# huakunyang/SummerTTS

Measured on AMD Instinct MI355X. Metric: audio samples/sec (acoustic model + vocoder, phoneme ids -> int16 PCM on host), single_speaker_fast-shaped synthetic blob, higher is better.
Workload: dtype f32 (decoder trunk convs AND the reverse flow's WaveNet convs (wn_flow.hip, one-utterance calls): fp32 operands as 2 fp16 terms = 22-23 of their 24 mantissa bits, 3 fp16 MFMA products per fp32 product, f32 accumulation -- measured error in `parity`, same tolerance as the exact-fp32 leg; batches addi

## Files before the change

summertts_amd/csrc/capi.hip:

```cpp
#include <stdlib.h>
#include <string.h>

#include <algorithm>
#include <new>
#include <string>
#include <vector>

#include "engine.hpp"
#include "eq_stream.hpp"
#include "join_stream.hpp"
#include "loud_stream.hpp"

using namespace sts;

struct sts_engine { Engine eng; };

static thread_local std::string g_err;
static int set_err(int code, const std::string& s) { g_err = s; return code; }

extern "C" {

const char* sts_last_error(void) { return g_err.c_str(); }
void sts_free(void* p) { free(p); }

// ... 643 lines not shown
    return STS_OK;
}
int sts_set_record_taps(sts_engine* e, int enable) { if (!e) return set_err(STS_EINVAL, "null engine"); e->eng.record_taps = enable != 0; return STS_OK; }
int sts_set_conv_math(sts_engine* e, int mode) {
    if (!e) return set_err(STS_EINVAL, "null engine");
    if (mode < 0 || mode > 3) return set_err(STS_EINVAL, "conv math: 0 = split-bf16 (default), 1 = exact fp32, 2 = split-bf16 wherever eligible, 3 = two-term fp16");
    e->eng.conv_math = mode;
    e->eng.h2_consecutive = 0; e->eng.h2_disabled = false;
    return STS_OK;
}
int sts_set_conv_mode(sts_engine* e, int mode) { if (!e) return set_err(STS_EINVAL, "null engine"); e->eng.conv_mode = mode; return STS_OK; }
int sts_debug_set(sts_engine* e, int key, int value) {
    if (!e) return set_err(STS_EINVAL, "null engine");
    switch (key) {
        case STS_DBG_ATTN_BLOCK_MIN_WGS: if (value < 1) return set_err(STS_EINVAL, "threshold must be >= 1"); e->eng.attn_block_min_wgs = value; return STS_OK;
        case STS_DBG_FLOW_FUSED: e->eng.flow_fused = value != 0; return STS_OK;
        case STS_DBG_LAUNCH_AHEAD: if (value < 0 || value > 2) return set_err(STS_EINVAL, "launch_ahead must be 0, 1 or 2"); if ((value == 2) != (e->eng.launch_ahead == 2)) { e->eng.seen_tf_.clear(); e->eng.seen_order_.clear(); } e->eng.launch_ahead = value; return STS_OK;
        case STS_DBG_H2P: e->eng.h2p = value < 0 ? 0 : (value > 4 ? 4 : value); return STS_OK;
        case STS_DBG_H2P_TILE: e->eng.h2p_tile = value; return STS_OK;
        case STS_DBG_CHAIN_STREAMS: e->eng.chain_streams_dbg = value; return STS_OK;
        case STS_DBG_TAIL_FUSED: e->eng.tail_fused = value != 0; return STS_OK;
        case STS_DBG_UPS_ROWPH: e->eng.ups_rowph = value != 0; return STS_OK;
        case STS_DBG_MEMO_CLEAR: e->eng.seen_tf_.clear(); e->eng.seen_order_.clear(); return STS_OK;
        case STS_DBG_ATTN_REG: e->eng.attn_reg = value != 0; return STS_OK;
        case STS_DBG_DDS_TAIL: e->eng.dds_tail = value != 0; return STS_OK;
        case STS_DBG_PCM_DIRECT: e->eng.pcm_direct = value != 0; return STS_OK;
        case STS_DBG_STREAM_RETRY_STEP: e->eng.stream_retry_step = value < 0 ? -1 : value; return STS_OK;
        case STS_DBG_STREAM_DIRECT: e->eng.stream_direct = value != 0; return STS_OK;
        case STS_DBG_POISON: e->eng.poison = (unsigned)value; return STS_OK;
        default: return set_err(STS_EINVAL, "unknown debug key");
    }
// ... 846 lines not shown
```

summertts_amd/csrc/engine.hip:

```cpp
#include "run_ctx.hpp"
#include <time.h>
#include "knobs.hpp"
#include "../../include/tts_logger.h"

#include <algorithm>
#include <chrono>
#include <math.h>
#include <stdlib.h>
#include <string.h>
#include <thread>

namespace sts {

Engine::~Engine() {
    if (stream) (void)hipStreamSynchronize(stream);
    free_model(model);
    if (arenaT_.base) (void)hipFree(arenaT_.base);
    if (arenaF_.base) (void)hipFree(arenaF_.base);
    if (pinned_) (void)hipHostFree(pinned_);
    if (pinned_pcm_) (void)hipHostFree(pinned_pcm_);
    if (d_rs_table) (void)hipFree(d_rs_table);
    if (loud_host_) (void)hipHostFree(loud_host_);
    if (lim_host_) (void)hipHostFree(lim_host_);
    if (d_eq_) (void)hipFree(d_eq_);
// ... 17 lines not shown
#elif defined(__aarch64__) || defined(__arm__)
    asm volatile("yield" ::: "memory");
#else
    std::this_thread::yield();
#endif
}

int Engine::init(const float* blob, int64_t bytes, int dev) {
    conv_math = default_conv_math();
    int count = 0;
    if (hipGetDeviceCount(&count) != hipSuccess || count <= 0)
        return fail(STS_EDEVICE, "no HIP device visible: the SummerTTS HIP engine needs an AMD GPU (gfx950) -- there is no CPU fallback");
    if (dev < 0 || dev >= count) return fail(STS_EINVAL, "device index out of range");
    device = dev;
    HIPCK(hipSetDevice(dev));
    HIPCK(hipStreamCreateWithFlags(&stream, hipStreamNonBlocking));
    for (auto& e : ev_) HIPCK(hipEventCreate(&e));
    HIPCK(hipEventCreateWithFlags(&ev_fork_, hipEventDisableTiming));
    HIPCK(hipEventCreateWithFlags(&ev_setup_, hipEventDisableTiming));
    for (auto& e : ev_join_) HIPCK(hipEventCreateWithFlags(&e, hipEventDisableTiming));
    {
        int lo = 0, hi = 0;
        (void)hipDeviceGetStreamPriorityRange(&lo, &hi);
        for (int k = 0; k < kAux; k++) {
            int pr = lo + (hi - lo) * k / (kAux > 1 ? kAux - 1 : 1);
            HIPCK(hipStreamCreateWithPriority(&aux_[k], hipStreamNonBlocking, pr));
        }
    }
    cur_ = stream;
    have_events_ = true;
// ... 879 lines not shown
    for (int u : M.up_rate) upS *= u;
    c.upS = upS;
    std::vector<size_t> stage_elems(M.n_up);
    size_t regA = 0, regB = 0;
    { int S = 1; for (int i = 0; i < M.n_up; i++) { S *= M.up_rate[i]; stage_elems[i] = (size_t)(3 + 4 * M.n_resk) * M.ups[i].Cout * Wcap * S;
          if (i & 1) { if (stage_elems[i] > regB) regB = stage_elems[i]; } else { if (stage_elems[i] > regA) regA = stage_elems[i]; } } }
    const long Lsb = c.Lsb = Wcap * upS + B;
    const int sbC = c.sbC = M.conv_post.Cout;
    bool use_ff = flow_fused && conv_mode == 0 && conv_math == 3 && !M.cp.empty() && wnH > 0;
    for (size_t i = 0; i < M.cp.size() && use_ff; i++)
        use_ff = M.cp[i].ff.ok && M.cp[i].wn.H == wnH && M.cp[i].wn.n == c.wnL && M.cp[i].ff.G == M.cp[0].ff.G && M.cp[i].wn.in[0].k == M.cp[0].wn.in[0].k;
    if (use_ff) {
        long tiles = 0;
        if (B == 1) tiles = (Ftot + 31) / 32;
        else for (int b = 0; b < B; b++) tiles += (p_lenF[b] + 31) / 32;
        use_ff = tiles * M.cp[0].ff.G <= 256;
    }
    c.use_ff = use_ff; c.ffG = use_ff ? M.cp[0].ff.G : 0;
    BufF& bf = c.bf;
    const OutChain& oc = c.oc;
    c.Ocap = oc.run[OS_RESAMPLE] ? out_count((long long)Wcap * hop) + B : (long long)Wcap * hop;
    if (c.join) c.Ocap = oc.run[OS_RESAMPLE] ? out_count(c.FJ * hop) + 1 : c.FJ * hop;
    const long long jwin = ss && c.join ? c.js.window_frames() * hop : c.FJ * hop;
    if (ss && c.join) c.Ocap = oc.run[OS_RESAMPLE] ? out_count(jwin) + 4 : jwin;
    if (ss && oc.run[OS_LIMIT] && oc.run[OS_RESAMPLE]) c.Ocap += B;
    pcm_in_host_ = pcm_direct && host_pcm && !ss && B == 1 && !record_taps && pinned_pcm_dev_ && (size_t)c.Ocap * 2 + 256 <= pinned_pcm_cap_ &&
                   (size_t)c.Ocap * 2 <= ((size_t)4 << 20);
    auto layoutF = [&](Arena& A) {
        A.used = 0;
        for (int q = 0; q < 2; q++) {
            bf.ff_h[q] = A.get<float>(use_ff ? (size_t)wnH * Ftot : 1);
// ... 128 lines not shown
                    }
                    A.w_pre = cp.pre.wh2; A.b_pre = cp.pre.bias; A.s_pre = cp.pre.h2_scale;
                    A.w_gate = ff.gate0; A.s_gate = ff.gate0_scale;
                } else {
                    A.h_in = bf.ff_h[(l - 1) & 1]; A.part_in = bf.ff_part[(l - 1) & 1]; A.part_n = G;
                    A.w_gate = w.in[l].wh2; A.s_gate = w.in[l].h2_scale;
                }
                A.part_stride = (long)((size_t)w.H * Ftot);
                A.h_out = bf.ff_h[l & 1]; A.part_out = bf.ff_part[l & 1];
                A.macc = bf.ff_macc[cs]; A.macc_stride = (long)hF; A.macc_init = l == 0;
                A.b_gate = w.in[l].bias;
                if (w.has_cond) { A.ubias = bt.cond_wn + (size_t)l * 2 * w.H * B; A.ubias_ld = B; }
                A.w_c = ff.wc[l]; A.s_c = ff.sc[l]; A.rows_c = ff.rows_c[l]; A.rows_res = ff.rows_res[l];
                A.b_res = ff.b_res[l]; A.b_m = ff.b_m;
                A.ovf = ovf_;
                flow_layer(A, stream);
                if (l == 0 && pend_set >= 0) { cur[x0h] = A.x0_out; pend_set = -1; }
            }
            ConvOpt os; os.epi = EPI_SUB;
            (void)conv_args(cp.post, nullptr, lv1, nullptr, lv1, os, nullptr);
            pend_set = cs; pend_half = x1h;
        }
        if (pend_set >= 0) finish_half(pend_half, pend_set);
        for (int hh = 0; hh < 2; hh++) if (cur[hh] != home[hh]) finish_half(hh, -1);
    } else
    {
    expand_frames(bt.m, Ttot, bt.cum, lvT.seg, lv1.seg, C, bf.z, Ftot, B, maxF, stream, &pnz);
    tap("z_p", bf.z, C, Ftot, Fcount);

    for (int i = M.n_flows - 1; i >= 0; i--) {
        const DCoupling& cp = M.cp[i];
// ... 502 lines not shown
```

summertts_amd/csrc/engine.hpp:

```cpp
#pragma once
#include <hip/hip_runtime.h>

#include <deque>
#include <map>
#include <unordered_map>
#include <string>
#include <vector>

#include "../../include/summertts_hip.h"
#include "kernels.hpp"
#include "model.hpp"

namespace sts {

struct Arena {
    char* base = nullptr; size_t cap = 0, used = 0; bool measuring = false;
    void* alloc(size_t bytes) {
        size_t a = (used + 255) & ~(size_t)255;
        used = a + bytes;
        if (measuring) return nullptr;
        return base + a;
    }
    template <typename T> T* get(size_t count) { return (T*)alloc(count * sizeof(T)); }
};
// ... 98 lines not shown
    long ahead_misses = 0;
    static constexpr size_t kMemoEntries = 1024;
    std::unordered_map<unsigned long long, long> seen_tf_; std::deque<unsigned long long> seen_order_;
    bool polite_wait = false;
    struct WaitEst { double us = 0.0; long phonemes = 0; };
    WaitEst wait_est_[2][24];
    void nap_before_wait(int which, long phonemes);
    void note_wait(int which, long phonemes, double waited_us, bool was_ready_at_wake);
    int final_sync(long phonemes);
    int ups_rowph = 1;
    int tail_fused = 1;
    int chain_streams_dbg = -1;
    int h2p = 1;
    int h2p_tile = -1;
    int flow_fused = 1;
    int stream_retry_step = -1;
    int stream_direct = 0;
    unsigned poison = 0;
    int64_t poison_bytes_ = 0;
    hipStream_t stream = nullptr;

private:
    int fail(int code, const std::string& msg) { err_ = msg; return code; }
    bool ensure(Arena& a, size_t bytes);
    bool ensure_pinned(size_t bytes);
    void poison_arena(const Arena& a);
    void poison_host16(void* p, size_t samples);
    void poison_host32(void* p, size_t words);
    ConvArgs conv_args(const DConv& c, const float* x, const Lvl& lin, float* y, const Lvl& lout, const ConvOpt& o, double* flops);
    void conv(const DConv& c, const float* x, const Lvl& lin, float* y, const Lvl& lout, const ConvOpt& o);
// ... 60 lines not shown
```

summertts_amd/csrc/kernels.hpp:

```cpp
#pragma once
#include <hip/hip_runtime.h>
#include <stdint.h>

#include <vector>

#include "../../include/summertts_hip.h"

namespace sts {

struct SegView {
    const int* off;
    const int* len;
    int scale;
    int extra;
    int ioff, ilen;
};

enum Epilogue : int {
    EPI_STORE = 0,
    EPI_RESADD = 1,
    EPI_SUB = 3,
    EPI_GATE = 4,
    EPI_RESSKIP = 5,
    EPI_TANH_PCM = 6,
// ... 103 lines not shown
    float* part_out;
    float* macc; long macc_stride; int macc_init;
    const void* w_gate; const float* b_gate; float s_gate;
    const float* ubias; int ubias_ld;
    const void* w_c; float s_c; int rows_c, rows_res;
    const float* b_res; const float* b_m;
    unsigned* ovf;
};
struct FlowFinishArgs {
    SegView seg; int B, max_len; int half;
    const float* src; long src_ld; float* dst; long dst_ld;
    const float* macc; int n; long macc_stride;
};
bool flow_layer_shape_ok(int H, int half, int k, int dil, int n_layers);
int flow_layer_groups(int H);
void flow_layer(const FlowLayerArgs& a, hipStream_t st);
void flow_finish(const FlowFinishArgs& a, hipStream_t st);

bool conv_mfma_eligible(const ConvArgs& a);
void conv_mfma(const ConvArgs& a, hipStream_t st, int tile = -1);
constexpr int kMaxGroup = 4;
struct ConvGroup { ConvArgs g[kMaxGroup]; int n; };
struct ResLayerArgs {
    const float* x; float* y;
    const float *w1, *b1, *w2, *b2;
    int k1, dil1, k2;
    const float *wu1, *wu2;
    const void *wb1, *wb2;
    float ws1, ws2;
};
struct ResLayerGroup {
// ... 239 lines not shown
```

summertts_amd/csrc/run_ctx.hpp:

```cpp
#pragma once
#include "engine.hpp"
#include "eq_stream.hpp"
#include "loud_stream.hpp"
#include "out_chain.hpp"
#include "join_stream.hpp"

namespace sts {

#define HIPCK(call)                                                                           \
    do {                                                                                      \
        hipError_t e__ = (call);                                                              \
        if (e__ != hipSuccess) return fail(STS_EDEVICE, std::string(#call) + ": " + hipGetErrorString(e__)); \
    } while (0)

struct BufT {
    int *meta_i; float* ls; float *ns, *nsw; uint64_t* seed; int* ids; int* forced;
    float *x, *qkv, *att, *y, *x1, *ffh, *m, *logs;
    float *dh, *dt1, *dt2, *dc, *dhh, *dp29, *dr[4], *dlogw;
    int *dur, *cum, *frames;
    float *g, *cond_dp, *cond_dec, *cond_wn;
    float* plan_rate; int *plan_fixed, *plan_target; long long* plan_rem; float* dur_w;
    int* mix;
    int *gain_q, *gain_h;
    int* join_sil;
// ... 42 lines not shown
    int *pm = nullptr, *p_offT = nullptr, *p_lenT = nullptr, *p_sid = nullptr, *p_offF = nullptr, *p_lenF = nullptr, *p_one = nullptr;
    int *d_offT = nullptr, *d_lenT = nullptr, *d_sid = nullptr, *d_offF = nullptr, *d_lenF = nullptr, *d_one = nullptr, *d_win = nullptr;
    bool inl = false, no_inline_seg = false, ms = false;
    long Ftot = 0; int maxF = 0, hop = 0;
    long Fld = 0; int maxFld = 0; bool ahead = false, ahead_b = false, mapped = false, forced = false;
    bool plan = false;
    bool gain = false;
    bool join = false;
    long long FJ = 0;
    bool mix = false;
    std::vector<Engine::Noise> nz; bool any_ns = false, any_nsw = false;
    std::vector<unsigned long long> req_keys; std::vector<long> predF;
    int halo = 0; long Wcap = 0; int upS = 1; long Lsb = 0; int sbC = 0;
    long long Ocap = 0;
    bool bstream = false;
    bool use_ff = false; int ffG = 0;
    OutChain oc{}; LimiterDesign limd; int rsP = 1, rsQ = 1, eqS = 0;
    const float* stage_out(int s) const {
        const float* const o[OS_COUNT] = {bf.wave, bf.wave_gain, bf.wave_join, bf.wave_out, nullptr, bf.wave_eq, nullptr, bf.wave_lim};
        return s < 0 ? nullptr : o[s];
    }
    JsPlan js;
};
#define RUN_ALIASES(c)                                                                                                              \
    [[maybe_unused]] Model& M = model;                                                                                              \
    [[maybe_unused]] const int B = (c).B; [[maybe_unused]] const StreamSpec* const ss = (c).ss;                                     \
    [[maybe_unused]] const long Ttot = (c).Ttot; [[maybe_unused]] const int maxT = (c).maxT;                                        \
    [[maybe_unused]] const int H = (c).H, C = (c).C, FF = (c).FF, fdp = (c).fdp, wnH = (c).wnH, wnL = (c).wnL, ffn2_slices = (c).ffn2_slices; \
    [[maybe_unused]] Lvl &lvT = (c).lvT, &lvB = (c).lvB, &lv1 = (c).lv1;                                                            \
    [[maybe_unused]] BufT& bt = (c).bt; [[maybe_unused]] BufF& bf = (c).bf;                                                         \
    [[maybe_unused]] const size_t up_bytes = (c).up_bytes;                                                                          \
// ... 12 lines not shown
```

summertts_amd/csrc/wn_flow.hip:

```cpp
#include "conv_bf3_dev.hpp"

namespace sts {

#ifdef STS_TILE_TRACE
int tile_trace_bind_flow(long long* buf, unsigned capacity_records) { return tile_trace_bind(buf, capacity_records); }
#endif

constexpr int FL_WIN = 64;
constexpr int FL_NT = 32;
constexpr int FL_UR = 2;
constexpr int FL_MAXG = 8;

__device__ __forceinline__ unsigned fl_b_off(int chunk, int pos, int half, int plane, int plane_bytes) {
    return (unsigned)(chunk * 2 * plane_bytes + plane * plane_bytes + pos * 32 + ((half ^ ((pos >> 3) & 1)) << 4));
}

__device__ __forceinline__ void split4h(const float (&x)[4], unsigned (&hi)[2], unsigned (&lo)[2], float& amax) {
#pragma unroll
    for (int d = 0; d < 2; d++) {
        const f32x2 v = {x[2 * d], x[2 * d + 1]};
        const f16x2 h = __builtin_convertvector(v, f16x2);
#if STS_SPLIT_MIX
        const f32x2 v2 = v * 2048.f;
        const unsigned hu = __builtin_bit_cast(unsigned, h);
// ... 3 lines not shown
            : "+v"(l) : "v"(hu), "s"(-2048.0f), "v"(v2[0]), "v"(v2[1]));
        hi[d] = hu;
        lo[d] = l;
#else
        const f32x2 r = (v - __builtin_convertvector(h, f32x2)) * 2048.f;
        const f16x2 l = __builtin_convertvector(r, f16x2);
        hi[d] = __builtin_bit_cast(unsigned, h);
        lo[d] = __builtin_bit_cast(unsigned, l);
#endif
        amax = __builtin_fmaxf(amax, __builtin_fmaxf(__builtin_fabsf(v[0]), __builtin_fabsf(v[1])));
    }
}

constexpr int FL_WAVES = 8;
constexpr int FL_GSTEPS = 16;
template <bool L0>
__global__ __launch_bounds__(64 * FL_WAVES) __attribute__((amdgpu_waves_per_eu(2, 2))) void flow_layer_kernel(FlowLayerArgs a) {
    extern __shared__ __attribute__((aligned(16))) unsigned char fsm[];
    const int Gp = (a.G + 7) & ~7;
    const int g = (int)(blockIdx.x % (unsigned)Gp);
    if (g >= a.G) return;
    const int rest = (int)(blockIdx.x / (unsigned)Gp);
    const int ntile = (a.max_len + FL_NT - 1) / FL_NT;
    const int b = rest / ntile, tile = rest - b * ntile;
    const int len = uni(seg_len(a.seg, b));
    const int n0 = tile * FL_NT;
    if (n0 >= len) return;
    const size_t base = (size_t)uni(seg_start(a.seg, b));
    const int tid = threadIdx.x, lane = tid & 63, wave = __builtin_amdgcn_readfirstlane(tid >> 6);
    const int l31 = lane & 31, half = lane >> 5;
    const int H = a.H, hc = a.half, Cg = a.Cg, halo = a.halo;
    const int W = FL_NT + 2 * halo;
    const int NCH = H >> 4;
    const int PLANE = FL_WIN * 32;
    unsigned char* const R_h = fsm;
    unsigned char* const R_x = fsm + (size_t)NCH * 2 * PLANE;
    unsigned char* const R_a = R_x + (size_t)FL_WAVES * 4096;
    const int APL = FL_NT * 32;
    float amax = 0.f;
    constexpr int RG = 2, KS = FL_WAVES / RG;
    const int rt_l = wave % RG, kq = wave / RG;
#ifdef STS_TILE_TRACE
    long long* tt_rec = tt_open(3 + (L0 ? 1 : 0), g);
    TT_STAMP(0);
#endif

    const int nrtg = (2 * H) >> 5;
    const int c_lo = NCH * kq / KS, c_hi = NCH * (kq + 1) / KS;
    const int nsteps = (c_hi - c_lo) * a.k;
    u32x4 fa[FL_GSTEPS][1][2];
    auto gate_prefetch = [&](auto lo_c, auto hi_c) {
        constexpr int lo = decltype(lo_c)::value, hi = decltype(hi_c)::value;
        const rsrc_t wrs = make_rsrc(a.w_gate, (unsigned)((size_t)NCH * a.k * nrtg * 2048u));
// ... 22 lines not shown
                    const unsigned off = t < ntc && cs < nkc ? (unsigned)(((g * nkc + cs) * ntc + t) * 2048 + pl * 1024 + lane * 16) : kOOB;
                    fc[ti][cs][0][pl] = __builtin_bit_cast(u32x4, __builtin_amdgcn_raw_buffer_load_b128(wrs, (int)off, 0, 0));
                }
        }
    };

    f32x4u mold[2][4];
    auto m_prefetch = [&]() {
        const rsrc_t rm = make_rsrc(a.macc + (size_t)g * a.macc_stride, a.macc_init ? 0u : (unsigned)(((size_t)a.tot * hc) * 4u));
#pragma unroll
        for (int ti = 0; ti < 2; ti++) {
            const int t = wave + FL_WAVES * ti;
#pragma unroll
            for (int q = 0; q < 4; q++) {
                const int c = t * 32 + 8 * q + 4 * half - a.rows_res;
                const bool okm = t < ntc && c >= 0 && c + 3 < hc && n0 + l31 < len;
                const unsigned off = okm ? (unsigned)(((base + (size_t)(n0 + l31)) * hc + c) * 4u) : kOOB;
                mold[ti][q] = __builtin_bit_cast(f32x4u, __builtin_amdgcn_raw_buffer_load_b128(rm, (int)off, 0, 0));
            }
        }
    };

    if constexpr (!L0) {
        gate_prefetch(I0{}, IH{});
        const int qpp = H >> 2;
        const int nunit = W * qpp;
        const unsigned span = (unsigned)(((size_t)a.tot * H) * 4u);
        const rsrc_t rh = make_rsrc(a.h_in, span);
        for (int u0 = 0; u0 < nunit; u0 += 64 * FL_WAVES * FL_UR) {
            f32x4u v[FL_UR], p[FL_UR][FL_MAXG];
            int pw[FL_UR], q4[FL_UR]; bool ok[FL_UR];
#pragma unroll
            for (int r = 0; r < FL_UR; r++) {
                const int u = u0 + r * 64 * FL_WAVES + tid;
                pw[r] = u / qpp; q4[r] = u - pw[r] * qpp;
                const int pos = n0 - halo + pw[r];
                ok[r] = u < nunit && pos >= 0 && pos < len;
                const unsigned off = ok[r] ? (unsigned)(((base + (size_t)pos) * H + (size_t)q4[r] * 4) * 4u) : kOOB;
                v[r] = __builtin_bit_cast(f32x4u, __builtin_amdgcn_raw_buffer_load_b128(rh, (int)off, 0, 0));
#pragma unroll
                for (int s = 0; s < FL_MAXG; s++) {
                    const rsrc_t rp = make_rsrc(a.part_in + (size_t)s * a.part_stride, s < a.part_n ? span : 0u);
                    p[r][s] = __builtin_bit_cast(f32x4u, __builtin_amdgcn_raw_buffer_load_b128(rp, (int)off, 0, 0));
                }
            }
#pragma unroll
            for (int r = 0; r < FL_UR; r++) {
                const int u = u0 + r * 64 * FL_WAVES + tid;
                if (u >= nunit) continue;
                f32x4u s4 = v[r];
#pragma unroll
                for (int s = 0; s < FL_MAXG; s++) s4 += p[r][s];
                const int ch = q4[r] * 4;
                if (ok[r] && pw[r] >= halo && pw[r] < halo + FL_NT && ch >= g * Cg && ch < (g + 1) * Cg)
                    *(f32x4u*)(a.h_out + (base + (size_t)(n0 - halo + pw[r])) * H + ch) = s4;
                const float x4[4] = {s4[0], s4[1], s4[2], s4[3]};
                unsigned hi[2], lo[2];
                split4h(x4, hi, lo, amax);
                const int chunk = ch >> 4, hf = (ch >> 3) & 1, qd = (ch >> 2) & 1;
                unsigned char* d = R_h + fl_b_off(chunk, pw[r], hf, 0, PLANE) + qd * 8;
                *(uint2*)d = uint2{hi[0], hi[1]};
                *(uint2*)(d + PLANE) = uint2{lo[0], lo[1]};
            }
        }
        TT_STAMP(1);
        gate_prefetch(IH{}, IE{});
        c_prefetch();
        m_prefetch();
    } else {
        gate_prefetch(I0{}, IH{});
        const int nrt = H >> 5, nk = hc >> 4;
        u32x4 fp[8][1][2];
        {
            const rsrc_t wrs = make_rsrc(a.w_pre, (unsigned)((size_t)nk * nrt * 2048u));
#pragma unroll
            for (int cs = 0; cs < 8; cs++)
#pragma unroll
                for (int pl = 0; pl < 2; pl++) {
                    const unsigned o = wave < nrt && cs < nk ? (unsigned)((cs * nrt + wave) * 2048 + pl * 1024 + lane * 16) : kOOB;
                    fp[cs][0][pl] = __builtin_bit_cast(u32x4, __builtin_amdgcn_raw_buffer_load_b128(wrs, (int)o, 0, 0));
                }
        }
        const int qpp = hc >> 2;
        const int nunit = W * qpp;
        const unsigned pspan = (unsigned)(((size_t)a.tot * hc) * 4u);
        for (int u0 = 0; u0 < nunit; u0 += 64 * FL_WAVES * FL_UR) {
            float zv[FL_UR][4]; f32x4u p[FL_UR][FL_MAXG];
            int pw[FL_UR], q4[FL_UR]; bool ok[FL_UR];
#pragma unroll
            for (int r = 0; r < FL_UR; r++) {
                const int u = u0 + r * 64 * FL_WAVES + tid;
                q4[r] = u / W; pw[r] = u - q4[r] * W;
                const int pos = n0 - halo + pw[r];
                ok[r] = u < nunit && pos >= 0 && pos < len;
                const size_t zo = (size_t)(q4[r] * 4) * a.x0_ld + base + (size_t)(ok[r] ? pos : 0);
#pragma unroll
                for (int e = 0; e < 4; e++) zv[r][e] = ok[r] ? a.x0[zo + (size_t)e * a.x0_ld] : 0.f;
                const unsigned off = ok[r] ? (unsigned)(((base + (size_t)pos) * hc + (size_t)q4[r] * 4) * 4u) : kOOB;
#pragma unroll
                for (int s = 0; s < FL_MAXG; s++) {
                    const rsrc_t rp = make_rsrc(a.pend + (size_t)s * a.pend_stride, s < a.pend_n ? pspan : 0u);
                    p[r][s] = __builtin_bit_cast(f32x4u, __builtin_amdgcn_raw_buffer_load_b128(rp, (int)off, 0, 0));
                }
            }
#pragma unroll
            for (int r = 0; r < FL_UR; r++) {
                const int u = u0 + r * 64 * FL_WAVES + tid;
                if (u >= nunit) continue;
                f32x4u s4 = {zv[r][0], zv[r][1], zv[r][2], zv[r][3]};
#pragma unroll
                for (int s = 0; s < FL_MAXG; s++) s4 += p[r][s];
                const int ch = q4[r] * 4;
                if (a.x0_out && ok[r] && pw[r] >= halo && pw[r] < halo + FL_NT && (q4[r] % a.G) == g) {
                    float* zp = a.x0_out + (size_t)ch * a.x0_out_ld + base + (size_t)(n0 - halo + pw[r]);
#pragma unroll
                    for (int e = 0; e < 4; e++) zp[(size_t)e * a.x0_out_ld] = s4[e];
                }
                const float x4[4] = {s4[0], s4[1], s4[2], s4[3]};
                unsigned hi[2], lo[2];
                split4h(x4, hi, lo, amax);
                const int chunk = ch >> 4, hf = (ch >> 3) & 1, qd = (ch >> 2) & 1;
                unsigned char* d = R_x + fl_b_off(chunk, pw[r], hf, 0, PLANE) + qd * 8;
                *(uint2*)d = uint2{hi[0], hi[1]};
                *(uint2*)(d + PLANE) = uint2{lo[0], lo[1]};
            }
        }
        __syncthreads();
        TT_STAMP(1);
        gate_prefetch(IH{}, IE{});
        if (wave < nrt) {
            const int rt = wave;
            f32x16 acc[1][2];
#pragma unroll
            for (int ct = 0; ct < 2; ct++)
#pragma unroll
                for (int r = 0; r < 16; r++) acc[0][ct][r] = 0.f;
#pragma unroll
            for (int cs = 0; cs < 8; cs++)
                if (cs < nk) {
                    u32x4 fb[2][2];
#pragma unroll
                    for (int ct = 0; ct < 2; ct++)
#pragma unroll
                        for (int pl = 0; pl < 2; pl++) fb[ct][pl] = *(const u32x4*)(R_x + fl_b_off(cs, ct * 32 + l31, half, pl, PLANE));
                    step_mfmas<1, 1, 2, 2, 2>(acc, fp[cs], fb);
                }
#pragma unroll
            for (int ct = 0; ct < 2; ct++) {
                const int pw_ = ct * 32 + l31;
                const int pos = n0 - halo + pw_;
                const bool inside = pos >= 0 && pos < len && pw_ < W;
#pragma unroll
                for (int hh = 0; hh < 2; hh++) {
                    float v8[8];
#pragma unroll
                    for (int e = 0; e < 8; e++) {
                        const int row = rt * 32 + hh * 16 + 8 * (e >> 2) + 4 * half + (e & 3);
                        const float t1 = acc[0][ct][hh * 8 + e] * a.s_pre + (a.b_pre ? a.b_pre[row] : 0.f);
                        v8[e] = inside ? t1 : 0.f;
                    }
                    u32x4 ph, pl;
                    split8h(v8, ph, pl, amax);
                    unsigned char* d = R_h + fl_b_off(rt * 2 + hh, pw_, half, 0, PLANE);
                    *(u32x4*)d = ph;
                    *(u32x4*)(d + PLANE) = pl;
                    if (inside && pw_ >= halo && pw_ < halo + FL_NT) {
#pragma unroll
                        for (int qd = 0; qd < 2; qd++) {
                            const int ch = rt * 32 + hh * 16 + 8 * qd + 4 * half;
                            if (ch >= g * Cg && ch < (g + 1) * Cg)
                                *(f32x4u*)(a.h_out + (base + (size_t)pos) * H + ch) = f32x4u{v8[4 * qd], v8[4 * qd + 1], v8[4 * qd + 2], v8[4 * qd + 3]};
                        }
                    }
                }
            }
        }
        c_prefetch();
        m_prefetch();
    }
    __syncthreads();
    TT_STAMP(2);

    f32x16 acc[1][1], acc1[1][1];
#pragma unroll
    for (int r = 0; r < 16; r++) { acc[0][0][r] = 0.f; acc1[0][0][r] = 0.f; }
    {
        u32x4 fb[2][1][2];
        auto load_b = [&](int s, u32x4 (&dst)[1][2]) {
            const int ss = s < nsteps ? s : 0;
            const int c = c_lo + ss / a.k, j = ss - (ss / a.k) * a.k;
// ... 8 lines not shown
                if constexpr (s % 2 == 0) step_mfmas<1, 1, 1, 2, 2>(acc, fa[s], fb[s % 2]);
                else step_mfmas<1, 1, 1, 2, 2>(acc1, fa[s], fb[s % 2]);
            }
        });
#pragma unroll
        for (int r = 0; r < 16; r++) acc[0][0][r] += acc1[0][0][r];
    }
    TT_STAMP(3);
    float* const red = (float*)R_x;
    __syncthreads();
#pragma unroll
    for (int r = 0; r < 16; r++) red[((size_t)(kq * RG + rt_l) * 16 + r) * 64 + lane] = acc[0][0][r];
    __syncthreads();
    {
        const int rowb = (g * RG + rt_l) * 32;
        float gv[2];
#pragma unroll
        for (int i = 0; i < 2; i++) {
            const int r = 2 * kq + i;
            float t = 0.f, sg = 0.f;
            for (int q = 0; q < KS; q++) {
                t += red[((size_t)(q * RG + rt_l) * 16 + r) * 64 + lane];
                sg += red[((size_t)(q * RG + rt_l) * 16 + r + 8) * 64 + lane];
            }
            const int rowp = rowb + (r & 3) + 8 * (r >> 2) + 4 * half;
            t = t * a.s_gate + (a.b_gate ? a.b_gate[rowp] : 0.f);
            sg = sg * a.s_gate + (a.b_gate ? a.b_gate[rowp + 16] : 0.f);
            if (a.ubias) { t += a.ubias[(size_t)rowp * a.ubias_ld + b]; sg += a.ubias[(size_t)(rowp + 16) * a.ubias_ld + b]; }
            gv[i] = tanh_ref(t) * sigmoid_ref(sg);
        }
        const f32x2 v = {gv[0], gv[1]};
        const f16x2 hh = __builtin_convertvector(v, f16x2);
        const f32x2 rr = (v - __builtin_convertvector(hh, f32x2)) * 2048.f;
        const f16x2 ll = __builtin_convertvector(rr, f16x2);
        amax = __builtin_fmaxf(amax, __builtin_fmaxf(__builtin_fabsf(v[0]), __builtin_fabsf(v[1])));
        unsigned char* d = R_a + (size_t)rt_l * 2 * APL + l31 * 32 + ((half ^ ((l31 >> 3) & 1)) << 4) + kq * 4;
        *(unsigned*)d = __builtin_bit_cast(unsigned, hh);
        *(unsigned*)(d + APL) = __builtin_bit_cast(unsigned, ll);
    }
    __syncthreads();
    TT_STAMP(4);

    const int pos_o = n0 + l31;
    const bool col_ok = pos_o < len;
#pragma unroll
    for (int ti = 0; ti < 2; ti++) {
        const int t = wave + FL_WAVES * ti;
        if (t >= ntc) continue;
        f32x16 ac[1][1];
#pragma unroll
        for (int r = 0; r < 16; r++) ac[0][0][r] = 0.f;
#pragma unroll
        for (int cs = 0; cs < 2; cs++)
            if (cs < nkc) {
                u32x4 fb[1][2];
                const unsigned char* sp = R_a + (size_t)cs * 2 * APL + l31 * 32 + ((half ^ ((l31 >> 3) & 1)) << 4);
                fb[0][0] = *(const u32x4*)sp;
                fb[0][1] = *(const u32x4*)(sp + APL);
                step_mfmas<1, 1, 1, 2, 2>(ac, fc[ti][cs], fb);
// ... 32 lines not shown
    const size_t base = (size_t)seg_start(a.seg, b);
    const int idx = blockIdx.x * 256 + threadIdx.x;
    const int qpp = a.half >> 2;
    const int q = idx / a.max_len, pos = idx - q * a.max_len;
    if (q >= qpp || pos >= len) return;
    f32x4u s4;
#pragma unroll
    for (int e = 0; e < 4; e++) s4[e] = a.src[(size_t)(q * 4 + e) * a.src_ld + base + pos];
    for (int s = 0; s < a.n; s++) s4 += *(const f32x4u*)(a.macc + (size_t)s * a.macc_stride + (base + (size_t)pos) * a.half + q * 4);
#pragma unroll
    for (int e = 0; e < 4; e++) a.dst[(size_t)(q * 4 + e) * a.dst_ld + base + pos] = s4[e];
}

bool flow_layer_shape_ok(int H, int half, int k, int dil, int n_layers) {
    if (H < 32 || H % 32 != 0 || H > 256 || half < 16 || half % 16 != 0 || half % 4 != 0 || half > 128) return false;
    if (!(k & 1) || k < 1 || dil != 1 || (k - 1) > FL_WIN - FL_NT || n_layers < 1) return false;
    const int Cg = 32, G = H / Cg;
    if (G > FL_MAXG) return false;
    const int RG = 2, KS = FL_WAVES / RG, NCH = H / 16;
    if (((NCH + KS - 1) / KS) * k > FL_GSTEPS) return false;
    if (half / 16 > 8 || H / 32 > FL_WAVES) return false;
    const int rows_c = ((H + half) + 31) / 32 * 32;
    return rows_c / 32 <= 2 * FL_WAVES;
}
int flow_layer_groups(int H) { return H / 32; }

static size_t flow_lds_bytes(int H) {
    const size_t h = (size_t)(H / 16) * 2 * FL_WIN * 32;
    return h + (size_t)FL_WAVES * 4096 + (size_t)4 * 2 * FL_NT * 32 + 256;
}

void flow_layer(const FlowLayerArgs& a, hipStream_t st) {
    if (a.max_len <= 0 || a.B <= 0) return;
    const int Gp = (a.G + 7) & ~7;
    const int ntile = (a.max_len + FL_NT - 1) / FL_NT;
    const size_t lds = flow_lds_bytes(a.H);
    if (a.layer == 0) {
        (void)hipFuncSetAttribute((const void*)flow_layer_kernel<true>, hipFuncAttributeMaxDynamicSharedMemorySize, (int)lds);
        hipLaunchKernelGGL(flow_layer_kernel<true>, dim3((unsigned)((size_t)ntile * a.B * Gp)), dim3(64 * FL_WAVES), lds, st, a);
    } else {
        (void)hipFuncSetAttribute((const void*)flow_layer_kernel<false>, hipFuncAttributeMaxDynamicSharedMemorySize, (int)lds);
        hipLaunchKernelGGL(flow_layer_kernel<false>, dim3((unsigned)((size_t)ntile * a.B * Gp)), dim3(64 * FL_WAVES), lds, st, a);
    }
}

void flow_finish(const FlowFinishArgs& a, hipStream_t st) {
    if (a.max_len <= 0 || a.B <= 0) return;
    const long n = (long)(a.half >> 2) * a.max_len;
    hipLaunchKernelGGL(flow_finish_kernel, dim3((unsigned)((n + 255) / 256), a.B), dim3(256), 0, st, a);
}

}
```

Baseline: 66.60 million.

## Add 16-column flow layer tiles for small utterances with compact block mapping

Templates the fused WaveNet flow layer kernel on its tile width and adds a 16-column variant. The engine picks it when the live tile count times the group count is at most half the CU count, so short one-utterance calls spread over more workgroups. The 16-wide path uses a denser block-to-(group, tile) mapping that does not waste padded group slots. The partial-sum accumulation loops are also specialised on the actual number of partials, so loads of absent slices are skipped. The cost is a second kernel instantiation and narrower MFMA work per block, which leaves half of each 32-column tile idle and recomputes halo more often.

```diff
diff --git a/summertts_amd/csrc/capi.hip b/summertts_amd/csrc/capi.hip
--- a/summertts_amd/csrc/capi.hip
+++ b/summertts_amd/csrc/capi.hip
@@ -681,7 +681,7 @@
     if (!e) return set_err(STS_EINVAL, "null engine");
     switch (key) {
         case STS_DBG_ATTN_BLOCK_MIN_WGS: if (value < 1) return set_err(STS_EINVAL, "threshold must be >= 1"); e->eng.attn_block_min_wgs = value; return STS_OK;
-        case STS_DBG_FLOW_FUSED: e->eng.flow_fused = value != 0; return STS_OK;
+        case STS_DBG_FLOW_FUSED: e->eng.flow_fused = value == 2 || value == 3 ? value : value != 0; return STS_OK;
         case STS_DBG_LAUNCH_AHEAD: if (value < 0 || value > 2) return set_err(STS_EINVAL, "launch_ahead must be 0, 1 or 2"); if ((value == 2) != (e->eng.launch_ahead == 2)) { e->eng.seen_tf_.clear(); e->eng.seen_order_.clear(); } e->eng.launch_ahead = value; return STS_OK;
         case STS_DBG_H2P: e->eng.h2p = value < 0 ? 0 : (value > 4 ? 4 : value); return STS_OK;
         case STS_DBG_H2P_TILE: e->eng.h2p_tile = value; return STS_OK;
diff --git a/summertts_amd/csrc/engine.hip b/summertts_amd/csrc/engine.hip
--- a/summertts_amd/csrc/engine.hip
+++ b/summertts_amd/csrc/engine.hip
@@ -55,6 +55,7 @@
     if (dev < 0 || dev >= count) return fail(STS_EINVAL, "device index out of range");
     device = dev;
     HIPCK(hipSetDevice(dev));
+    HIPCK(hipDeviceGetAttribute(&n_cus, hipDeviceAttributeMultiprocessorCount, dev));
     HIPCK(hipStreamCreateWithFlags(&stream, hipStreamNonBlocking));
     for (auto& e : ev_) HIPCK(hipEventCreate(&e));
     HIPCK(hipEventCreateWithFlags(&ev_fork_, hipEventDisableTiming));
@@ -964,7 +965,9 @@
         long tiles = 0;
         if (B == 1) tiles = (Ftot + 31) / 32;
         else for (int b = 0; b < B; b++) tiles += (p_lenF[b] + 31) / 32;
-        use_ff = tiles * M.cp[0].ff.G <= 256;
+        if (flow_fused < 2) use_ff = tiles * M.cp[0].ff.G <= 256;
+        const long live = B == 1 ? ((c.ahead && !c.predF.empty() ? c.predF[0] : c.Ftot) + 31) / 32 : tiles;
+        c.ffNT = flow_fused == 3 || (flow_fused == 1 && live * M.cp[0].ff.G <= n_cus / 2) ? 16 : 32;
     }
     c.use_ff = use_ff; c.ffG = use_ff ? M.cp[0].ff.G : 0;
     BufF& bf = c.bf;
@@ -1123,7 +1126,7 @@
                 A.w_c = ff.wc[l]; A.s_c = ff.sc[l]; A.rows_c = ff.rows_c[l]; A.rows_res = ff.rows_res[l];
                 A.b_res = ff.b_res[l]; A.b_m = ff.b_m;
                 A.ovf = ovf_;
-                flow_layer(A, stream);
+                flow_layer(A, stream, c.ffNT);
                 if (l == 0 && pend_set >= 0) { cur[x0h] = A.x0_out; pend_set = -1; }
             }
             ConvOpt os; os.epi = EPI_SUB;
diff --git a/summertts_amd/csrc/engine.hpp b/summertts_amd/csrc/engine.hpp
--- a/summertts_amd/csrc/engine.hpp
+++ b/summertts_amd/csrc/engine.hpp
@@ -136,6 +136,7 @@
     int h2p = 1;
     int h2p_tile = -1;
     int flow_fused = 1;
+    int n_cus = 0;
     int stream_retry_step = -1;
     int stream_direct = 0;
     unsigned poison = 0;
diff --git a/summertts_amd/csrc/kernels.hpp b/summertts_amd/csrc/kernels.hpp
--- a/summertts_amd/csrc/kernels.hpp
+++ b/summertts_amd/csrc/kernels.hpp
@@ -141,7 +141,7 @@
 };
 bool flow_layer_shape_ok(int H, int half, int k, int dil, int n_layers);
 int flow_layer_groups(int H);
-void flow_layer(const FlowLayerArgs& a, hipStream_t st);
+void flow_layer(const FlowLayerArgs& a, hipStream_t st, int nt = 32);
 void flow_finish(const FlowFinishArgs& a, hipStream_t st);
 
 bool conv_mfma_eligible(const ConvArgs& a);
diff --git a/summertts_amd/csrc/run_ctx.hpp b/summertts_amd/csrc/run_ctx.hpp
--- a/summertts_amd/csrc/run_ctx.hpp
+++ b/summertts_amd/csrc/run_ctx.hpp
@@ -80,7 +80,7 @@
     int halo = 0; long Wcap = 0; int upS = 1; long Lsb = 0; int sbC = 0;
     long long Ocap = 0;
     bool bstream = false;
-    bool use_ff = false; int ffG = 0;
+    bool use_ff = false; int ffG = 0, ffNT = 32;
     OutChain oc{}; LimiterDesign limd; int rsP = 1, rsQ = 1, eqS = 0;
     const float* stage_out(int s) const {
         const float* const o[OS_COUNT] = {bf.wave, bf.wave_gain, bf.wave_join, bf.wave_out, nullptr, bf.wave_eq, nullptr, bf.wave_lim};
diff --git a/summertts_amd/csrc/wn_flow.hip b/summertts_amd/csrc/wn_flow.hip
--- a/summertts_amd/csrc/wn_flow.hip
+++ b/summertts_amd/csrc/wn_flow.hip
@@ -6,8 +6,8 @@
 int tile_trace_bind_flow(long long* buf, unsigned capacity_records) { return tile_trace_bind(buf, capacity_records); }
 #endif
 
-constexpr int FL_WIN = 64;
-constexpr int FL_NT = 32;
+constexpr int FL_COLS = 32;
+constexpr int fl_win(int NT) { return NT + 32; }
 constexpr int FL_UR = 2;
 constexpr int FL_MAXG = 8;
 
@@ -41,14 +41,53 @@
 
 constexpr int FL_WAVES = 8;
 constexpr int FL_GSTEPS = 16;
-template <bool L0>
+
+#ifndef STS_FLOW_MAP
+#define STS_FLOW_MAP 0
+#endif
+__host__ __device__ __forceinline__ int flow_grid16(int G, int T) { return STS_FLOW_MAP == 1 ? T * G : 8 * G * ((T + 7) >> 3); }
+template <class F>
+__device__ __forceinline__ void fl_slices(int n, F&& f) {
+    switch (n) {
+        case 0: f(std::integral_constant<int, 0>{}); break;
+        case 1: f(std::integral_constant<int, 1>{}); break;
+        case 2: f(std::integral_constant<int, 2>{}); break;
+        case 3: f(std::integral_constant<int, 3>{}); break;
+        case 4: f(std::integral_constant<int, 4>{}); break;
+        case 5: f(std::integral_constant<int, 5>{}); break;
+        case 6: f(std::integral_constant<int, 6>{}); break;
+        case 7: f(std::integral_constant<int, 7>{}); break;
+        default: f(std::integral_constant<int, 8>{}); break;
+    }
+}
+__device__ __forceinline__ bool flow_block_map(int bid, int G, int T, int& g, int& rest) {
+#if STS_FLOW_MAP == 1
+    rest = bid / G; g = bid - rest * G;
+#else
+    const int c = bid & 7, s = bid >> 3;
+    const int q = s / G, i = s - q * G;
+    if (c < G) { g = c; rest = 8 * q + i; }
+    else {
+        const int m = (c - G) * G + i, sp = 8 - G;
+        g = m / sp; rest = 8 * q + G + (m - g * sp);
+    }
+#endif
+    return rest < T;
+}
+template <bool L0, int NT>
 __global__ __launch_bounds__(64 * FL_WAVES) __attribute__((amdgpu_waves_per_eu(2, 2))) void flow_layer_kernel(FlowLayerArgs a) {
     extern __shared__ __attribute__((aligned(16))) unsigned char fsm[];
-    const int Gp = (a.G + 7) & ~7;
-    const int g = (int)(blockIdx.x % (unsigned)Gp);
-    if (g >= a.G) return;
-    const int rest = (int)(blockIdx.x / (unsigned)Gp);
+    constexpr int FL_NT = NT, FL_WIN = fl_win(NT);
     const int ntile = (a.max_len + FL_NT - 1) / FL_NT;
+    int g, rest;
+    if constexpr (NT == 32) {
+        const int Gp = (a.G + 7) & ~7;
+        g = (int)(blockIdx.x % (unsigned)Gp);
+        if (g >= a.G) return;
+        rest = (int)(blockIdx.x / (unsigned)Gp);
+    } else {
+        if (!flow_block_map((int)blockIdx.x, a.G, ntile * a.B, g, rest)) return;
+    }
     const int b = rest / ntile, tile = rest - b * ntile;
     const int len = uni(seg_len(a.seg, b));
     const int n0 = tile * FL_NT;
@@ -63,7 +102,7 @@
     unsigned char* const R_h = fsm;
     unsigned char* const R_x = fsm + (size_t)NCH * 2 * PLANE;
     unsigned char* const R_a = R_x + (size_t)FL_WAVES * 4096;
-    const int APL = FL_NT * 32;
+    constexpr int APL = FL_COLS * 32;
     float amax = 0.f;
     constexpr int RG = 2, KS = FL_WAVES / RG;
     const int rt_l = wave % RG, kq = wave / RG;
@@ -116,7 +155,7 @@
 #pragma unroll
             for (int q = 0; q < 4; q++) {
                 const int c = t * 32 + 8 * q + 4 * half - a.rows_res;
-                const bool okm = t < ntc && c >= 0 && c + 3 < hc && n0 + l31 < len;
+                const bool okm = t < ntc && c >= 0 && c + 3 < hc && l31 < FL_NT && n0 + l31 < len;
                 const unsigned off = okm ? (unsigned)(((base + (size_t)(n0 + l31)) * hc + c) * 4u) : kOOB;
                 mold[ti][q] = __builtin_bit_cast(f32x4u, __builtin_amdgcn_raw_buffer_load_b128(rm, (int)off, 0, 0));
             }
@@ -129,8 +168,10 @@
         const int nunit = W * qpp;
         const unsigned span = (unsigned)(((size_t)a.tot * H) * 4u);
         const rsrc_t rh = make_rsrc(a.h_in, span);
+        fl_slices(a.part_n, [&](auto ns_c) {
+        constexpr int NS = decltype(ns_c)::value;
         for (int u0 = 0; u0 < nunit; u0 += 64 * FL_WAVES * FL_UR) {
-            f32x4u v[FL_UR], p[FL_UR][FL_MAXG];
+            f32x4u v[FL_UR], p[FL_UR][NS > 0 ? NS : 1];
             int pw[FL_UR], q4[FL_UR]; bool ok[FL_UR];
 #pragma unroll
             for (int r = 0; r < FL_UR; r++) {
@@ -141,8 +182,8 @@
                 const unsigned off = ok[r] ? (unsigned)(((base + (size_t)pos) * H + (size_t)q4[r] * 4) * 4u) : kOOB;
                 v[r] = __builtin_bit_cast(f32x4u, __builtin_amdgcn_raw_buffer_load_b128(rh, (int)off, 0, 0));
 #pragma unroll
-                for (int s = 0; s < FL_MAXG; s++) {
-                    const rsrc_t rp = make_rsrc(a.part_in + (size_t)s * a.part_stride, s < a.part_n ? span : 0u);
+                for (int s = 0; s < NS; s++) {
+                    const rsrc_t rp = make_rsrc(a.part_in + (size_t)s * a.part_stride, span);
                     p[r][s] = __builtin_bit_cast(f32x4u, __builtin_amdgcn_raw_buffer_load_b128(rp, (int)off, 0, 0));
                 }
             }
@@ -152,7 +193,8 @@
                 if (u >= nunit) continue;
                 f32x4u s4 = v[r];
 #pragma unroll
-                for (int s = 0; s < FL_MAXG; s++) s4 += p[r][s];
+                for (int s = 0; s < NS; s++) s4 += p[r][s];
+                if constexpr (NS < FL_MAXG) s4 += f32x4u{0.f, 0.f, 0.f, 0.f};
                 const int ch = q4[r] * 4;
                 if (ok[r] && pw[r] >= halo && pw[r] < halo + FL_NT && ch >= g * Cg && ch < (g + 1) * Cg)
                     *(f32x4u*)(a.h_out + (base + (size_t)(n0 - halo + pw[r])) * H + ch) = s4;
@@ -165,6 +207,7 @@
                 *(uint2*)(d + PLANE) = uint2{lo[0], lo[1]};
             }
         }
+        });
         TT_STAMP(1);
         gate_prefetch(IH{}, IE{});
         c_prefetch();
@@ -186,8 +229,10 @@
         const int qpp = hc >> 2;
         const int nunit = W * qpp;
         const unsigned pspan = (unsigned)(((size_t)a.tot * hc) * 4u);
+        fl_slices(a.pend_n, [&](auto ns_c) {
+        constexpr int NS = decltype(ns_c)::value;
         for (int u0 = 0; u0 < nunit; u0 += 64 * FL_WAVES * FL_UR) {
-            float zv[FL_UR][4]; f32x4u p[FL_UR][FL_MAXG];
+            float zv[FL_UR][4]; f32x4u p[FL_UR][NS > 0 ? NS : 1];
             int pw[FL_UR], q4[FL_UR]; bool ok[FL_UR];
 #pragma unroll
             for (int r = 0; r < FL_UR; r++) {
@@ -200,8 +245,8 @@
                 for (int e = 0; e < 4; e++) zv[r][e] = ok[r] ? a.x0[zo + (size_t)e * a.x0_ld] : 0.f;
                 const unsigned off = ok[r] ? (unsigned)(((base + (size_t)pos) * hc + (size_t)q4[r] * 4) * 4u) : kOOB;
 #pragma unroll
-                for (int s = 0; s < FL_MAXG; s++) {
-                    const rsrc_t rp = make_rsrc(a.pend + (size_t)s * a.pend_stride, s < a.pend_n ? pspan : 0u);
+                for (int s = 0; s < NS; s++) {
+                    const rsrc_t rp = make_rsrc(a.pend + (size_t)s * a.pend_stride, pspan);
                     p[r][s] = __builtin_bit_cast(f32x4u, __builtin_amdgcn_raw_buffer_load_b128(rp, (int)off, 0, 0));
                 }
             }
@@ -211,7 +256,8 @@
                 if (u >= nunit) continue;
                 f32x4u s4 = {zv[r][0], zv[r][1], zv[r][2], zv[r][3]};
 #pragma unroll
-                for (int s = 0; s < FL_MAXG; s++) s4 += p[r][s];
+                for (int s = 0; s < NS; s++) s4 += p[r][s];
+                if constexpr (NS < FL_MAXG) s4 += f32x4u{0.f, 0.f, 0.f, 0.f};
                 const int ch = q4[r] * 4;
                 if (a.x0_out && ok[r] && pw[r] >= halo && pw[r] < halo + FL_NT && (q4[r] % a.G) == g) {
                     float* zp = a.x0_out + (size_t)ch * a.x0_out_ld + base + (size_t)(n0 - halo + pw[r]);
@@ -227,28 +273,30 @@
                 *(uint2*)(d + PLANE) = uint2{lo[0], lo[1]};
             }
         }
+        });
         __syncthreads();
         TT_STAMP(1);
         gate_prefetch(IH{}, IE{});
-        if (wave < nrt) {
+        auto pre_park = [&](auto nct_c) {
+            constexpr int NCT = decltype(nct_c)::value;
             const int rt = wave;
-            f32x16 acc[1][2];
-#pragma unroll
-            for (int ct = 0; ct < 2; ct++)
+            f32x16 acc[1][NCT];
+#pragma unroll
+            for (int ct = 0; ct < NCT; ct++)
 #pragma unroll
                 for (int r = 0; r < 16; r++) acc[0][ct][r] = 0.f;
 #pragma unroll
             for (int cs = 0; cs < 8; cs++)
                 if (cs < nk) {
-                    u32x4 fb[2][2];
-#pragma unroll
-                    for (int ct = 0; ct < 2; ct++)
+                    u32x4 fb[NCT][2];
+#pragma unroll
+                    for (int ct = 0; ct < NCT; ct++)
 #pragma unroll
                         for (int pl = 0; pl < 2; pl++) fb[ct][pl] = *(const u32x4*)(R_x + fl_b_off(cs, ct * 32 + l31, half, pl, PLANE));
-                    step_mfmas<1, 1, 2, 2, 2>(acc, fp[cs], fb);
-                }
-#pragma unroll
-            for (int ct = 0; ct < 2; ct++) {
+                    step_mfmas<1, 1, NCT, 2, 2>(acc, fp[cs], fb);
+                }
+#pragma unroll
+            for (int ct = 0; ct < NCT; ct++) {
                 const int pw_ = ct * 32 + l31;
                 const int pos = n0 - halo + pw_;
                 const bool inside = pos >= 0 && pos < len && pw_ < W;
@@ -276,6 +324,9 @@
                     }
                 }
             }
+        };
+        if (wave < nrt) {
+            pre_park(std::integral_constant<int, FL_NT < 32 ? 1 : 2>{});
         }
         c_prefetch();
         m_prefetch();
@@ -314,35 +365,47 @@
     __syncthreads();
     {
         const int rowb = (g * RG + rt_l) * 32;
-        float gv[2];
-#pragma unroll
-        for (int i = 0; i < 2; i++) {
-            const int r = 2 * kq + i;
+        auto gated = [&](int r, int src) {
             float t = 0.f, sg = 0.f;
             for (int q = 0; q < KS; q++) {
-                t += red[((size_t)(q * RG + rt_l) * 16 + r) * 64 + lane];
-                sg += red[((size_t)(q * RG + rt_l) * 16 + r + 8) * 64 + lane];
+                t += red[((size_t)(q * RG + rt_l) * 16 + r) * 64 + src];
+                sg += red[((size_t)(q * RG + rt_l) * 16 + r + 8) * 64 + src];
             }
             const int rowp = rowb + (r & 3) + 8 * (r >> 2) + 4 * half;
             t = t * a.s_gate + (a.b_gate ? a.b_gate[rowp] : 0.f);
             sg = sg * a.s_gate + (a.b_gate ? a.b_gate[rowp + 16] : 0.f);
             if (a.ubias) { t += a.ubias[(size_t)rowp * a.ubias_ld + b]; sg += a.ubias[(size_t)(rowp + 16) * a.ubias_ld + b]; }
-            gv[i] = tanh_ref(t) * sigmoid_ref(sg);
-        }
-        const f32x2 v = {gv[0], gv[1]};
-        const f16x2 hh = __builtin_convertvector(v, f16x2);
-        const f32x2 rr = (v - __builtin_convertvector(hh, f32x2)) * 2048.f;
-        const f16x2 ll = __builtin_convertvector(rr, f16x2);
-        amax = __builtin_fmaxf(amax, __builtin_fmaxf(__builtin_fabsf(v[0]), __builtin_fabsf(v[1])));
-        unsigned char* d = R_a + (size_t)rt_l * 2 * APL + l31 * 32 + ((half ^ ((l31 >> 3) & 1)) << 4) + kq * 4;
-        *(unsigned*)d = __builtin_bit_cast(unsigned, hh);
-        *(unsigned*)(d + APL) = __builtin_bit_cast(unsigned, ll);
+            return tanh_ref(t) * sigmoid_ref(sg);
+        };
+        if constexpr (FL_NT == FL_COLS) {
+            float gv[2];
+#pragma unroll
+            for (int i = 0; i < 2; i++) gv[i] = gated(2 * kq + i, lane);
+            const f32x2 v = {gv[0], gv[1]};
+            const f16x2 hh = __builtin_convertvector(v, f16x2);
+            const f32x2 rr = (v - __builtin_convertvector(hh, f32x2)) * 2048.f;
+            const f16x2 ll = __builtin_convertvector(rr, f16x2);
+            amax = __builtin_fmaxf(amax, __builtin_fmaxf(__builtin_fabsf(v[0]), __builtin_fabsf(v[1])));
+            unsigned char* d = R_a + (size_t)rt_l * 2 * APL + l31 * 32 + ((half ^ ((l31 >> 3) & 1)) << 4) + kq * 4;
+            *(unsigned*)d = __builtin_bit_cast(unsigned, hh);
+            *(unsigned*)(d + APL) = __builtin_bit_cast(unsigned, ll);
+        } else {
+            const int i = l31 >> 4, col = l31 & 15;
+            float v = gated(2 * kq + i, (lane & 32) | col);
+            asm("" : "+v"(v));
+            const _Float16 hh = (_Float16)v;
+            const _Float16 ll = (_Float16)((v - (float)hh) * 2048.f);
+            amax = __builtin_fmaxf(amax, __builtin_fabsf(v));
+            unsigned char* d = R_a + (size_t)rt_l * 2 * APL + col * 32 + ((half ^ ((col >> 3) & 1)) << 4) + kq * 4 + i * 2;
+            *(_Float16*)d = hh;
+            *(_Float16*)(d + APL) = ll;
+        }
     }
     __syncthreads();
     TT_STAMP(4);
 
     const int pos_o = n0 + l31;
-    const bool col_ok = pos_o < len;
+    const bool col_ok = l31 < FL_NT && pos_o < len;
 #pragma unroll
     for (int ti = 0; ti < 2; ti++) {
         const int t = wave + FL_WAVES * ti;
@@ -405,7 +468,7 @@
 
 bool flow_layer_shape_ok(int H, int half, int k, int dil, int n_layers) {
     if (H < 32 || H % 32 != 0 || H > 256 || half < 16 || half % 16 != 0 || half % 4 != 0 || half > 128) return false;
-    if (!(k & 1) || k < 1 || dil != 1 || (k - 1) > FL_WIN - FL_NT || n_layers < 1) return false;
+    if (!(k & 1) || k < 1 || dil != 1 || (k - 1) > 16 || n_layers < 1) return false;
     const int Cg = 32, G = H / Cg;
     if (G > FL_MAXG) return false;
     const int RG = 2, KS = FL_WAVES / RG, NCH = H / 16;
@@ -416,22 +479,29 @@
 }
 int flow_layer_groups(int H) { return H / 32; }
 
-static size_t flow_lds_bytes(int H) {
-    const size_t h = (size_t)(H / 16) * 2 * FL_WIN * 32;
-    return h + (size_t)FL_WAVES * 4096 + (size_t)4 * 2 * FL_NT * 32 + 256;
-}
-
-void flow_layer(const FlowLayerArgs& a, hipStream_t st) {
+static size_t flow_lds_bytes(int H, int nt) {
+    const size_t h = (size_t)(H / 16) * 2 * fl_win(nt) * 32;
+    return h + (size_t)FL_WAVES * 4096 + (size_t)4 * 2 * FL_COLS * 32 + 256;
+}
+
+template <bool L0, int NT>
+static void flow_layer_launch(const FlowLayerArgs& a, unsigned grid, hipStream_t st) {
+    const size_t lds = flow_lds_bytes(a.H, NT);
+    (void)hipFuncSetAttribute((const void*)flow_layer_kernel<L0, NT>, hipFuncAttributeMaxDynamicSharedMemorySize, (int)lds);
+    hipLaunchKernelGGL((flow_layer_kernel<L0, NT>), dim3(grid), dim3(64 * FL_WAVES), lds, st, a);
+}
+
+void flow_layer(const FlowLayerArgs& a, hipStream_t st, int nt) {
     if (a.max_len <= 0 || a.B <= 0) return;
-    const int Gp = (a.G + 7) & ~7;
-    const int ntile = (a.max_len + FL_NT - 1) / FL_NT;
-    const size_t lds = flow_lds_bytes(a.H);
-    if (a.layer == 0) {
-        (void)hipFuncSetAttribute((const void*)flow_layer_kernel<true>, hipFuncAttributeMaxDynamicSharedMemorySize, (int)lds);
-        hipLaunchKernelGGL(flow_layer_kernel<true>, dim3((unsigned)((size_t)ntile * a.B * Gp)), dim3(64 * FL_WAVES), lds, st, a);
+    if (nt == 16) {
+        const unsigned grid = (unsigned)flow_grid16(a.G, (a.max_len + 15) / 16 * a.B);
+        if (a.layer == 0) flow_layer_launch<true, 16>(a, grid, st);
+        else flow_layer_launch<false, 16>(a, grid, st);
     } else {
-        (void)hipFuncSetAttribute((const void*)flow_layer_kernel<false>, hipFuncAttributeMaxDynamicSharedMemorySize, (int)lds);
-        hipLaunchKernelGGL(flow_layer_kernel<false>, dim3((unsigned)((size_t)ntile * a.B * Gp)), dim3(64 * FL_WAVES), lds, st, a);
+        const int Gp = (a.G + 7) & ~7;
+        const unsigned grid = (unsigned)((size_t)((a.max_len + 31) / 32) * a.B * Gp);
+        if (a.layer == 0) flow_layer_launch<true, 32>(a, grid, st);
+        else flow_layer_launch<false, 32>(a, grid, st);
     }
 }
 
```

Measured after the change: 67.33 million, median of 6. 1.1% higher.
